# shaneson0/attacking_federate_learning

Measured on AMD Instinct MI355X. Metric: aggregation rounds/sec at N clients x D params (Bulyan), higher is better.
Workload: dtype f32 (Gram: fp16x2 split of every fp32 operand, 3 fp16 MFMAs per block, fp32/fp64 accumulate; <= 2e-7 of |gi||gj| vs f...

## Files before the change

### attacking_federate_learning_amd/_native.py

```python
import ctypes
import os

_HERE = os.path.dirname(os.path.abspath(__file__))
LIB_PATH = os.environ.get('BYZ_LIBRARY') or os.path.join(_HERE, 'libbyzagg.so')

OK, E_INVALID, E_PRECONDITION, E_HIP, E_UNSUPPORTED, E_NO_WINNER, E_COLLECTIVE = 0, -1, -2, -3, -4, -5, -6

KERNELS = ('column_stats', 'gram_tile', 'gram_reduce', 'distances', 'row_sort', 'krum_argmin',
           'bulyan_loop', 'trimmed_mean', 'misc', 'plane_split')

c_i64, c_i32, c_int, c_f32, c_vp = ctypes.c_int64, ctypes.c_int32, ctypes.c_int, ctypes.c_float, ctypes.c_void_p
_P = ctypes.POINTER



class GeomedParams(ctypes.Structure):
    _fields_ = [('nu', ctypes.c_double), ('max_iter', c_i64), ('ftol', ctypes.c_double)]


class CclipParams(ctypes.Structure):
    _fields_ = [('tau', ctypes.c_double), ('iters', c_i64)]


SIGNGUARD_MAX_SAMPLES = 1024
# ... 59 lines not shown
    'byz_upload': [c_vp, c_vp, c_vp, c_i64, c_vp],
    'byz_download': [c_vp, c_vp, c_vp, c_i64, c_vp],
    'byz_upload_2d': [c_vp, c_vp, c_i64, c_vp, c_i64, c_i64, c_i64, c_vp],
    'byz_stream_sync': [c_vp, c_vp],
    'byz_no_defense_dev': [c_vp, c_vp, c_i64, c_i64, c_i64, c_vp, c_vp],
    'byz_pairwise_distances_dev': [c_vp, c_vp, c_i64, c_i64, c_i64, c_vp, c_vp],
    'byz_gram_dev': [c_vp, c_vp, c_i64, c_i64, c_i64, c_vp, c_vp],
    'byz_gram_share_dev': [c_vp, c_vp, c_i64, c_i64, c_i64, c_vp, c_int, c_int, c_vp, c_vp],
    'byz_gram_share_add_dev': [c_vp, c_vp, c_i64, c_i64, c_i64, c_vp, c_int, c_int, c_vp, c_vp],
    'byz_distances_from_gram_dev': [c_vp, c_vp, c_i64, c_vp, c_vp],
    'byz_near_pairs_count': [c_vp, _P(c_i64), c_vp],
    'byz_near_pairs_sqdist_dev': [c_vp, c_vp, c_i64, c_i64, c_i64, c_vp, c_vp, c_vp],
    'byz_near_pairs_apply_dev': [c_vp, c_vp, c_i64, c_vp, c_vp],
    'byz_ctx_check': [c_vp, c_vp],
    'byz_bulyan_rescored': [c_vp, _P(c_i64)],
    'byz_krum_select_dev': [c_vp, c_vp, c_i64, c_i64, c_i64, _P(c_i32), c_vp, c_vp],
    'byz_krum_dev': [c_vp, c_vp, c_i64, c_i64, c_i64, c_i64, c_i64, c_int, c_vp, _P(c_i32), c_vp],
    'byz_trimmed_mean_dev': [c_vp, c_vp, c_i64, c_i64, c_i64, c_vp, c_i64, c_vp, c_vp],
    'byz_coordinate_median_dev': [c_vp, c_vp, c_i64, c_i64, c_i64, c_vp, c_vp, c_vp],
    'byz_rank_trimmed_mean_dev': [c_vp, c_vp, c_i64, c_i64, c_i64, c_vp, c_i64, c_vp, c_vp],
    'byz_window_mean_dev': [c_vp, c_vp, c_i64, c_i64, c_i64, c_vp, c_vp, c_i64, c_vp, c_vp, c_vp],
    'byz_phocas_dev': [c_vp, c_vp, c_i64, c_i64, c_i64, c_vp, c_i64, c_vp, c_vp, c_vp, c_vp],
    'byz_trimmed_mean_redone': [c_vp, _P(c_i64), c_vp],
    'byz_bulyan_select_dev': [c_vp, c_vp, c_i64, c_i64, c_i64, c_vp, c_vp],
    'byz_krum_bulyan_select_dev': [c_vp, c_vp, c_i64, c_i64, c_i64, _P(c_i32), c_vp, c_vp],
    'byz_bulyan_dev': [c_vp, c_vp, c_i64, c_i64, c_i64, c_i64, c_i64, c_vp, c_vp, c_vp],
    'byz_mean_rows_dev': [c_vp, c_vp, c_i64, c_i64, c_i64, c_vp, c_i64, c_vp, c_vp],
    'byz_multi_krum_select_dev': [c_vp, c_vp, c_i64, c_i64, c_i64, c_i64, c_vp, c_vp],
    'byz_multi_krum_dev': [c_vp, c_vp, c_i64, c_i64, c_i64, c_i64, c_i64, c_i64, c_int, c_vp, c_vp, c_vp],
    'byz_pairwise_distances_sharded_dev': [c_vp, c_vp, c_i64, c_i64, c_i64, c_vp, c_vp, c_vp, c_vp],
# ... 191 lines not shown
```

### attacking_federate_learning_amd/csrc/api.hip

```cpp
#include "common.hpp"

#include <cmath>
#include <cstring>

namespace byz {

static thread_local char g_error[1024] = "";

void set_error(const char* fmt, ...) {
    va_list ap;
    va_start(ap, fmt);
    vsnprintf(g_error, sizeof(g_error), fmt, ap);
    va_end(ap);
}

namespace {

int64_t python_prefix_len(int64_t length, int64_t stop) {
    if (stop >= 0) return stop < length ? stop : length;
    return length + stop > 0 ? length + stop : 0;
}

int enter(byz_ctx* ctx) {
    if (!ctx) {
// ... 190 lines not shown
    if (theta < 0 || theta > n) {
        set_error("bulyan: selection size %lld does not fit %lld rows", (long long)theta, (long long)n);
        return BYZ_E_INVALID;
    }
    int64_t drop = (n - 1) - users_count + corrupted;
    if (drop < 0) drop = 0;
    if (drop > n - 1) drop = n - 1;
    const int64_t krum_prefix = krum_winner_dev != nullptr ? python_prefix_len(n - 1, users_count - corrupted) : 0;
    BYZ_TRY(launch_row_sort(ctx, dist, n, krum_prefix, drop, true, stream));
    if (krum_winner_dev != nullptr) BYZ_TRY(launch_krum_argmin(ctx, n, krum_winner_dev, stream));
    BYZ_TRY(launch_bulyan_loop(ctx, dist, n, theta, drop, users_count, corrupted, selection_dev, &device_scalars(ctx)->core.bulyan, stream));
    CoreScalars core;
    BYZ_TRY(read_core(ctx, &core, stream));
    const int32_t status = core.bulyan.status;
    ctx->bulyan_rescored = core.bulyan.rescored;
    if (status == 2) {
        set_error("bulyan: the selection loop's workgroups lost contact with each other (exchange timed out)");
        return BYZ_E_HIP;
    }
    if (status != 0) {
        set_error("bulyan: no row scored below 1e20 (the reference raises KeyError(-1) here)");
        return BYZ_E_NO_WINNER;
    }
    return BYZ_OK;
}

int check_multi_krum_m(int64_t n, int64_t m) {
    if (m < 1 || m > n) {
        set_error("multi_krum: m = %lld outside 1..%lld (the row count)", (long long)m, (long long)n);
        return BYZ_E_INVALID;
// ... 280 lines not shown
    BYZ_REQUIRE(sq_dev && dist && n_rows > 0 && ctx->near_pair_capacity > 0, "near_pairs_apply: bad arguments");
    return launch_near_pair_apply(ctx, sq_dev, n_rows, dist, as_stream(stream));
}

int byz_ctx_check(byz_ctx* ctx, void* stream) {
    BYZ_TRY(enter(ctx));
    return check_core(ctx, as_stream(stream));
}

int byz_bulyan_rescored(const byz_ctx* ctx, int64_t* rows_host) {
    if (!ctx || !rows_host) {
        set_error("bulyan_rescored: null argument");
        return BYZ_E_INVALID;
    }
    *rows_host = ctx->bulyan_rescored;
    return BYZ_OK;
}

int byz_pairwise_distances_dev(byz_ctx* ctx, const float* G, int64_t n_rows, int64_t n_cols, int64_t ld,
                               float* dist, void* stream) {
    BYZ_TRY(enter(ctx));
    BYZ_TRY(check_matrix(G, n_rows, n_cols, ld, "pairwise_distances"));
    BYZ_REQUIRE(dist, "pairwise_distances: null output");
    return distances(ctx, G, n_rows, n_cols, ld, nullptr, nullptr, dist, stream);
}

int byz_krum_select_dev(byz_ctx* ctx, const float* dist, int64_t n_rows, int64_t users_count,
                        int64_t corrupted_count, int32_t* index_host, float* scores_dev, void* stream) {
    BYZ_TRY(enter(ctx));
    BYZ_REQUIRE(dist && n_rows > 0, "krum_select: bad arguments");
// ... 2532 lines not shown
```

### attacking_federate_learning_amd/csrc/common.hpp

```cpp
#pragma once

#include <hip/hip_runtime.h>

#include <cstdarg>
#include <cstdint>
#include <cstdio>
#include <cstdlib>
#include <string>
#include <unordered_map>
#include <vector>

#include "../../include/byzagg.h"
#include "carve.hpp"
#include "device_scalars.hpp"

namespace byz {

void set_error(const char* fmt, ...);

#define BYZ_HIP(expr)                                                                       \
    do {                                                                                    \
        hipError_t e_ = (expr);                                                             \
        if (e_ != hipSuccess) {                                                             \
            ::byz::set_error("%s failed: %s (%s:%d)", #expr, hipGetErrorString(e_), __FILE__, \
// ... 130 lines not shown
    int64_t fang_steps = 0, fang_chosen = -1;
    int32_t fang_succeeded = 0;
    byz::Buffer phocas;
    byz::Buffer large_keys;
    byz::Buffer large_idx;
    byz::Buffer large_rank;
    byz::Buffer large_rank_t;
    byz::Buffer large_dist_t;
    byz::Buffer large_state;
    byz::Buffer large_grid;
    bool redo_valid = false;
    byz::Buffer redo_tiles;
    byz::Buffer twin_class;
    byz::Buffer xchg;
    int64_t bulyan_rescored = 0;
    byz::Buffer selection;
    byz::Buffer scalars;
    byz::LastCall last[byz::kReportCount];
    bool small_configured = false;
    std::unordered_map<const void*, int> dynamic_lds;
    byz::Buffer assemble_table;
    std::vector<int64_t> assemble_host;
    hipEvent_t assemble_copied = nullptr;
    int64_t assemble_clients = 0, assemble_segments = 0, assemble_longest = 0, assemble_total = 0;
    byz::Buffer stage_in;
    byz::Buffer stage_out;
    byz::PinnedBuffer pinned;
    bool timing = false;
    byz::TimingSlot slots[BYZ_K_COUNT];
};
// ... 325 lines not shown
```

### attacking_federate_learning_amd/csrc/device_scalars.hpp

```cpp
#pragma once

#include <hip/hip_runtime.h>

#include <cstddef>
#include <cstdint>
#include <type_traits>

namespace byz {

constexpr int kStatusLostTicket = 1;
constexpr int kStatusPairOverflow = 2;
constexpr int kStatusFalseTwin = 4;
constexpr int kStatusSmallTimeout = 8;
constexpr int kStatusNoTurn = 16;

struct BulyanStatus { int32_t status, rescored, pad; };
struct CoreScalars {
    int32_t krum_winner, pad0[7];
    BulyanStatus bulyan;
    int32_t pad1[5];
    int32_t status;
    int32_t near_pairs;
    int32_t attack_redo, pad2;
};
struct GeomedReport {
    int32_t done, iterations, excluded, fallback;
    double objective;
};
struct DncReport { int32_t kept, inactive; };
struct CclipReport { int32_t clipped, excluded; };
struct FltrustReport {
// ... 108 lines not shown
```

### attacking_federate_learning_amd/csrc/select.hip

```cpp
#include "common.hpp"
#include "lane_exchange.hpp"
#include "order_keys.hpp"

#include <cstdlib>
#include <cstring>

namespace byz {
namespace {

using namespace lanes;

constexpr int kMaxSelectRows = 16384;
constexpr float kKrumInit = 1e20f;

__device__ __forceinline__ float integer_passes(uint32_t (&M)[8], const int (&ex)[8], float s, int lane);

__device__ __forceinline__ int sort_slot(int i) { return i + (i >> 4); }

__device__ __forceinline__ double key_to_double(uint32_t ordered, uint32_t column) {
    return static_cast<double>((static_cast<unsigned long long>(ordered) << 16) | column);
}
__device__ __forceinline__ unsigned long long double_to_key(double d) {
    const unsigned long long x = static_cast<unsigned long long>(d);
    return ((x >> 16) << 32) | (x & 0xffffull);
// ... 728 lines not shown
    int u, bad, ptr, alive;

    __device__ __forceinline__ void init(int row, int n, int drop, const double* __restrict__ row_total, const double* __restrict__ row_top,
                                         const uint16_t* __restrict__ rank_t, float* sorted_val) {
        u = row;
        alive = u < n;
        tot = alive ? row_total[u] : 0.0;
        top = (alive && drop > 0) ? row_top[u] : 0.0;
        bad = alive ? static_cast<int>(row_top[n + u]) : 0;
        ptr = n - 1 - drop;
        if (alive) sorted_val[static_cast<int64_t>(u) * n + rank_t[static_cast<int64_t>(u) * n + u]] = __uint_as_float(kGoneBits);
    }

    __device__ __forceinline__ void remove(int w, int n, int drop, const float* __restrict__ dist, const uint16_t* __restrict__ sorted_idx,
                                           const uint16_t* __restrict__ rank_t, const uint32_t* removed) {
        if (!alive) return;
        if (u == w) {
            alive = 0;
            return;
        }
        const float dwf = dist[static_cast<int64_t>(w) * n + u];
        const bool dw_finite = __builtin_fabsf(dwf) <= 3.4028234663852886e38f;
        const double dw = dw_finite ? static_cast<double>(dwf) : 0.0;
        if (!dw_finite) --bad;
        const int r = rank_t[static_cast<int64_t>(w) * n + u];
        tot -= dw;
        if (drop > 0 && r >= ptr) {
            top -= dw;
            int p = ptr - 1;
            const uint16_t* order = sorted_idx + static_cast<int64_t>(u) * n;
            while (p >= 0) {
                const int col = order[p];
                if (!((removed[col >> 5] >> (col & 31)) & 1u)) break;
                --p;
            }
            if (p >= 0) {
                const float joins = dist[static_cast<int64_t>(u) * n + order[p]];
                if (__builtin_fabsf(joins) <= 3.4028234663852886e38f) top += static_cast<double>(joins);
            }
            ptr = p;
        }
    }
};

__global__ __launch_bounds__(kGridThreads) void bulyan_grid_kernel(
    const float* __restrict__ dist, int n, int theta, int drop, int users_count, int corrupted,
    const uint16_t* __restrict__ sorted_idx, const uint16_t* __restrict__ rank_t, float* sorted_val,
    const double* __restrict__ row_total, const double* __restrict__ row_top, const int32_t* __restrict__ cls,
// ... 196 lines not shown
                    }
                    ptr = p;
                }
            }
        }
    }
    if (tid == 0) {
        if (result != 0) atomicMax(status, result);
        if (n_rescored) atomicAdd(rescored, n_rescored);
    }
}


constexpr int kSpecMax = 32;
constexpr int kSpecTable = 512;

__global__ __launch_bounds__(kGridThreads) void spec_owner_kernel(const double* __restrict__ row_total, const double* __restrict__ row_top,
                                                                  const int32_t* __restrict__ cls, int n, int drop, int n_wgs,
                                                                  int32_t* __restrict__ owner) {
    static_assert(kGridThreads == 256, "four waves per workgroup");
    __shared__ double tile[kGridThreads];
    __shared__ int copy[kGridThreads];
    __shared__ int sums[3][64];
    const int tid = threadIdx.x, lane = tid & 63, part = tid >> 6;
    const int u = blockIdx.x * 64 + lane;
    auto first_score = [&](int v) -> double {
        if (v >= n) return __builtin_inf();
        const double s = row_total[v] - (drop > 0 ? row_top[v] : 0.0);
        return s == s ? s : __builtin_inf();
    };
    const double su = first_score(u);
    const bool u_copy = u < n && cls[u] != u;
    int rank = 0, copies = 0, copies_before = 0;
    if (tid < 64) sums[0][tid] = sums[1][tid] = sums[2][tid] = 0;
    for (int v0 = 0; v0 < n; v0 += kGridThreads) {
        tile[tid] = first_score(v0 + tid);
        copy[tid] = (v0 + tid < n && cls[v0 + tid] != v0 + tid) ? 1 : 0;
        __syncthreads();
        const int m = n - v0 < kGridThreads ? n - v0 : kGridThreads;
        const int j_end = 64 * part + 64 < m ? 64 * part + 64 : m;
#pragma unroll 8
        for (int j = 64 * part; j < j_end; ++j) {
            const double sv = tile[j];
            const int cj = copy[j];
            copies += cj;
            copies_before += (cj != 0 && v0 + j < u) ? 1 : 0;
            rank += (cj == 0 && (sv < su || (sv == su && v0 + j < u))) ? 1 : 0;
        }
        __syncthreads();
    }
    atomicAdd(&sums[0][lane], rank);
    atomicAdd(&sums[1][lane], copies);
    atomicAdd(&sums[2][lane], copies_before);
    __syncthreads();
    if (part != 0 || u >= n) return;
    rank = sums[0][lane];
    copies = sums[1][lane];
    copies_before = sums[2][lane];
    if (u_copy) {
        owner[copies_before] = u;
        return;
    }
    const int q = copies / kGridThreads, rem = copies % kGridThreads;
    const int narrow = n_wgs - q - 1, wide = n_wgs - q;
    const int first_part = rem * narrow;
    int wg, local;
    if (rank < first_part) {
        local = rank / narrow;
        wg = q + 1 + rank % narrow;
    } else {
        const int r = rank - first_part;
        local = rem + r / wide;
        wg = q + r % wide;
    }
    owner[wg * kGridThreads + local] = u;
}

struct SpecVerdict {
    int k_bad;
    int winner;
    int timeout;
};

template <int kSpecThreads>
__global__ __launch_bounds__(kSpecThreads) void bulyan_spec_kernel(
    const float* __restrict__ dist, int n, int theta, int drop, int users_count, int corrupted,
    const uint16_t* __restrict__ sorted_idx, const uint16_t* __restrict__ rank_t, float* sorted_val,
    const double* __restrict__ row_total, const double* __restrict__ row_top, const int32_t* __restrict__ cls,
    unsigned long long* __restrict__ xchg, int32_t* __restrict__ selection, int32_t* __restrict__ status,
    int32_t* __restrict__ rescored, int batch_picks, const int32_t* __restrict__ owner) {
    __shared__ __attribute__((aligned(16))) float rescore_stage[kSpecThreads / 64][512];
    __shared__ Candidate slots[kSpecThreads / 64];
    __shared__ double second_slots[kSpecThreads / 64];
    __shared__ uint32_t removed[kMaxSelectRows / 32];
    __shared__ __attribute__((aligned(16))) uint32_t egone[kSpecThreads / 64][kMaxSelectRows / 32];
    __shared__ GridDecision decision;
    __shared__ int decision_contested;
    __shared__ unsigned long long leader_of[kSpecTable];
    __shared__ uint16_t items[kGridThreads * kSpecMax];
    __shared__ int n_items;
    __shared__ Candidate wave_bests[kSpecThreads / 64][kSpecMax];
    __shared__ int winners[kSpecMax];
    __shared__ SpecVerdict verdict;
    __shared__ int true_row[kSpecMax];
    __shared__ uint16_t front_batches[kGridThreads];
    const int tid = threadIdx.x, lane = tid & 63, wave = tid >> 6;
    const int n_wgs = gridDim.x, wg = blockIdx.x;
    const int u = tid < kGridThreads ? owner[wg * kGridThreads + tid] : n;
    for (int i = tid; i < kMaxSelectRows / 32; i += kSpecThreads) {
        removed[i] = 0u;
#pragma unroll
        for (int w = 0; w < kSpecThreads / 64; ++w) egone[w][i] = 0u;
    }
    if (tid < kGridThreads) front_batches[tid] = 0;

    BulyanRow row;
    row.init(u, n, drop, row_total, row_top, rank_t, sorted_val);
    const int my_class = row.alive ? cls[u] : 0;
    const int my_pos = visit_position(u);
    int n_rescored = 0;
    __syncthreads();

    auto slot = [&](int parity, int kind) { return xchg + (parity * 3 + kind) * kGridMaxWgs; };
    auto batch_slot = [&](int parity, int k) { return xchg + (6 + parity * kSpecMax + k) * kGridMaxWgs; };
    const unsigned long long none_a = (static_cast<unsigned long long>(kInfBits) << 32) | (static_cast<unsigned long long>(kNoRow) << 18);

    auto remove_winner = [&](int w) __attribute__((always_inline)) {
        if (tid == 0) removed[w >> 5] |= 1u << (w & 31);
        __syncthreads();
        row.remove(w, n, drop, dist, sorted_idx, rank_t, removed);
    };

    int result = (n < 2 && theta > 0) ? 1 : 0;
    int t = 0;
    uint32_t seq = 0;
    uint32_t batch_seq = 0;
    while (t < theta && result == 0) {
        const BulyanRow snapshot = row;
        const int t0 = t;
        const int kmax = theta - t0 < batch_picks ? theta - t0 : batch_picks;
        uint32_t cmask = 0;
        uint32_t contested = 0;
        int n_done = 0, pending = 0;
        for (int k = 0; k < kmax; ++k, ++seq) {
            const int tt = t0 + k;
            const uint32_t tag = ((seq >> 1) & 7u) + 1u;
            const uint32_t tag18 = (seq + 1u) & 0x3ffffu;
            const int parity = static_cast<int>(seq & 1u);
            const int take = take_at(tt, n, users_count, corrupted);
            const double score = row.tot - row.top;
            const bool candidate = row.alive && row.bad <= drop && score < static_cast<double>(kKrumInit);
            Candidate c{static_cast<double>(kKrumInit), 0x7fffffff, -1, -1};
            if (candidate) c = Candidate{score, my_pos, u, my_class};
            const Candidate best = block_best_dpp(c, slots);
            const int best_class = best.cls;
            double second = (candidate && my_class != best_class) ? score : __builtin_inf();
            second = wave_min_dpp(second);
            if (lane == 0) second_slots[wave] = second;
            __syncthreads();
// ... 10 lines not shown
                unsigned long long gb = static_cast<unsigned long long>(__float_as_uint(b_lb)) << 32;
                bool ok = true;
                if (n_wgs > 1) {
                    if (lane == 0) {
                        granule_store(slot(parity, 0) + wg, ga | tag);
                        granule_store(slot(parity, 1) + wg, gb | tag18);
                    }
                    unsigned long long va = none_a, vb = static_cast<unsigned long long>(kInfBits) << 32;
                    ok = gather_granule_pair(slot(parity, 0), slot(parity, 1), n_wgs, tag, tag18, lane, va, vb);
                    ga = va;
                    gb = vb;
                } else if (lane != 0) {
                    ga = none_a;
                    gb = static_cast<unsigned long long>(kInfBits) << 32;
                }
                const float a = __uint_as_float(static_cast<uint32_t>(ga >> 32));
                const float b = __uint_as_float(static_cast<uint32_t>(gb >> 32));
                const int a_row = static_cast<int>((ga >> 18) & 0x3fffu);
                const int a_cls = static_cast<int>((ga >> 4) & 0x3fffu);
                const float m1 = wave_min_dpp(a);
                GridDecision d{0, -1, 0.0};
                int is_contested = 0;
                if (!ok) {
                    d.mode = 3;
                } else if (!(m1 < __builtin_inff())) {
                    d.mode = 2;
                } else {
                    const double thr = band_threshold(m1, take);
                    d.threshold = thr;
                    const bool in_a = static_cast<double>(a) <= thr;
                    const bool in_b = static_cast<double>(b) <= thr;
                    const unsigned long long first = __ballot(a == m1);
                    const int lead_cls = __builtin_amdgcn_readlane(a_cls, __builtin_ctzll(first));
                    const bool one_class = __ballot(in_b) == 0ull && __ballot(in_a && a_cls != lead_cls) == 0ull;
                    const int pos = wave_min_dpp((one_class ? in_a : a == m1) ? visit_position(a_row) : 0x7fffffff);
                    d.winner = row_of_visit(pos);
                    is_contested = one_class ? 0 : 1;
                }
                if (lane == 0) {
                    decision = d;
                    decision_contested = is_contested;
                }
            }
            __syncthreads();
            const GridDecision d = decision;
            if (d.mode == 3) {
                result = 2;
                break;
            }
            if (d.mode == 2) {
                pending = 1;
                ++seq;
                break;
            }
            if (decision_contested != 0) {
                contested |= 1u << k;
                if (candidate && score <= d.threshold) cmask |= 1u << k;
            }
            if (tid == 0) winners[k] = d.winner;
            remove_winner(d.winner);
            ++n_done;
        }
        if (result != 0) break;
        contested &= n_done >= 32 ? ~0u : (1u << n_done) - 1u;
        cmask &= contested;

        int k_bad = -1, w_true = -1;
        if (contested != 0u) {
            for (int i = tid; i < kSpecTable; i += kSpecThreads) leader_of[i] = ~0ull;
            if (tid == 0) n_items = 0;
            if (tid < (kSpecThreads / 64) * kSpecMax)
                (&wave_bests[0][0])[tid] = Candidate{static_cast<double>(kKrumInit), 0x7fffffff, -1, -1};
            __syncthreads();
            for (uint32_t m = cmask; m != 0u; m &= m - 1u) {
                const int k = __builtin_ctz(m);
                const unsigned long long key = (static_cast<unsigned long long>(my_pos) << 32) | (static_cast<uint32_t>(k) << 16) | static_cast<uint32_t>(my_class);
// ... 104 lines not shown
                    }
                    verdict = v;
                }
                __syncthreads();
            }
            ++batch_seq;
            if (verdict.timeout != 0) {
                result = 2;
                break;
            }
            k_bad = verdict.k_bad;
            w_true = verdict.winner;
        }
        if (k_bad >= 0) {
            row = snapshot;
            __syncthreads();
            if (tid == 0) {
                for (int k = 0; k < n_done; ++k) removed[winners[k] >> 5] &= ~(1u << (winners[k] & 31));
                if (w_true >= 0) winners[k_bad] = w_true;
            }
            __syncthreads();
            n_done = w_true >= 0 ? k_bad + 1 : k_bad;
            pending = w_true >= 0 ? 0 : 1;
            for (int k = 0; k < n_done; ++k) remove_winner(winners[k]);
        }
        __syncthreads();
        for (int k = 0; k < n_done; ++k) {
            const int w = winners[k];
            if (wg == 0 && tid == 0) selection[t0 + k] = w;
            if (row.alive) sorted_val[static_cast<int64_t>(u) * n + rank_t[static_cast<int64_t>(w) * n + u]] = __uint_as_float(kGoneBits);
        }
        t = t0 + n_done;
        if (pending != 0) result = 1;
        __syncthreads();
    }
    if (tid == 0) {
        if (result != 0) atomicMax(status, result);
        if (n_rescored) atomicAdd(rescored, n_rescored);
    }
}

}

int64_t select_max_rows() { return kLargeMaxRows; }

bool select_large_applies(int64_t n) {
    if (n > kMaxSelectRows) return true;
    const char* e = std::getenv("BYZ_SELECT_LARGE");
    return e != nullptr && std::atoi(e) != 0;
}

int launch_row_sort(byz_ctx* ctx, const float* dist, int64_t n, int64_t prefix_len, int64_t drop_count,
                    bool want_tables, hipStream_t stream) {
// ... 47 lines not shown
    return check_launch("row_sort_kernel");
}

int launch_krum_argmin(byz_ctx* ctx, int64_t n, int32_t* winner_dev, hipStream_t stream) {
    KernelTimer t(ctx, BYZ_K_KRUM_ARGMIN, stream);
    krum_argmin_kernel<<<1, 1024, 0, stream>>>(ctx->scores.as<float>(), (int)n, winner_dev);
    return check_launch("krum_argmin_kernel");
}

int launch_bulyan_loop(byz_ctx* ctx, const float* dist, int64_t n, int64_t theta, int64_t drop_count,
                       int64_t users_count, int64_t corrupted, int32_t* selection_dev, BulyanStatus* status_dev,
                       hipStream_t stream) {
    BYZ_REQUIRE(dist && selection_dev && status_dev && n > 0 && theta >= 0 && theta <= n,
                "bulyan loop: bad arguments (n=%lld theta=%lld)", (long long)n, (long long)theta);
    BYZ_TRY(ctx->twin_class.ensure(static_cast<size_t>(2 * n) * sizeof(int32_t)));
    constexpr size_t kGranules = static_cast<size_t>(2 * 3 + 2 * kSpecMax) * kGridMaxWgs;
    BYZ_TRY(ctx->xchg.ensure(kGranules * sizeof(unsigned long long)));
    int32_t* cls_tmp = ctx->twin_class.as<int32_t>();
    int32_t* cls = cls_tmp + n;
    BYZ_HIP(hipMemsetAsync(ctx->xchg.ptr, 0, kGranules * sizeof(unsigned long long), stream));
    BYZ_HIP(hipMemsetAsync(status_dev, 0, sizeof *status_dev, stream));
    KernelTimer t(ctx, BYZ_K_BULYAN_LOOP, stream);
    twin_class_kernel<<<static_cast<unsigned>(ceil_div(n, 4)), 256, 0, stream>>>(dist, (int)n, cls_tmp);
    BYZ_TRY(check_launch("twin_class_kernel"));
    twin_class_fix_kernel<<<static_cast<unsigned>(ceil_div(n, 256)), 256, 0, stream>>>(cls_tmp, (int)n, cls);
    BYZ_TRY(check_launch("twin_class_fix_kernel"));
    if (select_large_applies(n))
        return launch_bulyan_loop_large(ctx, dist, n, theta, drop_count, users_count, corrupted, cls, selection_dev, status_dev, stream);
    const unsigned n_wgs = static_cast<unsigned>(ceil_div(n, kGridThreads));
    int batch = n >= 6000 ? 16 : (n >= 1000 ? 32 : 0);
    if (const char* e = std::getenv("BYZ_BULYAN_BATCH")) batch = std::atoi(e);
    if (batch > kSpecMax) batch = kSpecMax;
    if (batch >= 1) {
        BYZ_TRY(ctx->spec_owner.ensure(static_cast<size_t>(n_wgs) * kGridThreads * sizeof(int32_t)));
        int32_t* owner = ctx->spec_owner.as<int32_t>();
        BYZ_HIP(hipMemsetD32Async(reinterpret_cast<hipDeviceptr_t>(owner), static_cast<int>(n), static_cast<size_t>(n_wgs) * kGridThreads, stream));
        spec_owner_kernel<<<static_cast<unsigned>(ceil_div(n, 64)), kGridThreads, 0, stream>>>(
            ctx->row_total.as<double>(), ctx->row_top.as<double>(), cls, (int)n, (int)drop_count, (int)n_wgs, owner);
        BYZ_TRY(check_launch("spec_owner_kernel"));
        auto* spec = n >= 6000 ? &bulyan_spec_kernel<512> : &bulyan_spec_kernel<256>;
        spec<<<n_wgs, n >= 6000 ? 512 : 256, 0, stream>>>(
            dist, (int)n, (int)theta, (int)drop_count, (int)users_count, (int)corrupted, ctx->sorted_idx.as<uint16_t>(),
            ctx->rank_t.as<uint16_t>(), ctx->sorted_val.as<float>(), ctx->row_total.as<double>(), ctx->row_top.as<double>(), cls,
            ctx->xchg.as<unsigned long long>(), selection_dev, &status_dev->status, &status_dev->rescored, batch, owner);
        return check_launch("bulyan_spec_kernel");
    }
    bulyan_grid_kernel<<<n_wgs, kGridThreads, 0, stream>>>(
        dist, (int)n, (int)theta, (int)drop_count, (int)users_count, (int)corrupted, ctx->sorted_idx.as<uint16_t>(),
        ctx->rank_t.as<uint16_t>(), ctx->sorted_val.as<float>(), ctx->row_total.as<double>(), ctx->row_top.as<double>(), cls,
        ctx->xchg.as<unsigned long long>(), selection_dev, &status_dev->status, &status_dev->rescored);
    return check_launch("bulyan_grid_kernel");
}

}
```

### attacking_federate_learning_amd/engine.py

```python
import ctypes
import itertools
import os

import numpy as np

from . import _native

NAME_TO_ID = {'NoDefense': 0, 'Krum': 1, 'TrimmedMean': 2, 'Bulyan': 3}


def dnc_columns(n_cols, sub_dim, n_iters=1, seed=0):
    n_cols, sub_dim, n_iters = int(n_cols), int(sub_dim), int(n_iters)
    if n_iters < 1 or sub_dim < 1 or n_cols < 1:
        raise ValueError('dnc_columns: n_iters, sub_dim and n_cols must be >= 1')
    rng = np.random.default_rng(seed)
    rows = []
    for _ in range(n_iters):
        if sub_dim >= n_cols:
            rows.append(np.arange(n_cols, dtype=np.int64))
        else:
            rows.append(np.sort(rng.choice(n_cols, sub_dim, replace=False)).astype(np.int64))
    return np.stack(rows)


# ... 709 lines not shown

    def krum_bulyan_select(self, distances, users_count, corrupted_count, on_device=False):
        theta = int(users_count) - 2 * int(corrupted_count)
        with _Call(self) as c:
            d, keys = c.distances(distances)
            sel = DeviceBuffer(self, (max(theta, 1),), np.int32)
            idx = ctypes.c_int32(-2)
            c.run(self.lib.byz_krum_bulyan_select_dev(self.ctx, d.ptr, d.n, int(users_count), int(corrupted_count),
                                                      ctypes.byref(idx), sel.ptr, None), reads_back=True)
            index = int(idx.value)
            index = index if (keys is None or index < 0) else keys[index]
            return index, self._selection(sel, theta, keys, on_device)

    def bulyan_rescored(self):
        return self._read(self.lib.byz_bulyan_rescored, [ctypes.c_int64])[0]

    def bulyan(self, g, users_count, corrupted_count, return_selection=False):
        assert users_count >= 4 * corrupted_count + 3
        dm = self._device_matrix(g)
        if dm is None:
            if return_selection:
                out, aux = self.defend_host('Bulyan', g, users_count, corrupted_count, want_aux=True)
                return out, aux[:int(users_count) - 2 * int(corrupted_count)]
            return self.defend_host('Bulyan', g, users_count, corrupted_count)
        theta = int(users_count) - 2 * int(corrupted_count)
        with _Call(self) as c:
            m = c.matrix(dm)
            out, ptr = c.out(m.cols)
            sel, sel_ptr = c.out(max(theta, 1), np.int32, want=return_selection)
            c.run(self.lib.byz_bulyan_dev(self.ctx, m.ptr, m.rows, m.cols, m.ld, int(users_count), int(corrupted_count), ptr,
# ... 1587 lines not shown
```

### include/byzagg.h

```cpp
#ifndef BYZAGG_H
#define BYZAGG_H

#include <stdint.h>

#ifdef __cplusplus
extern "C" {
#endif

#define BYZ_ABI_VERSION 1

enum {
    BYZ_OK = 0,
    BYZ_E_INVALID = -1,
    BYZ_E_PRECONDITION = -2,
    BYZ_E_HIP = -3,
    BYZ_E_UNSUPPORTED = -4,
    BYZ_E_NO_WINNER = -5,
    BYZ_E_COLLECTIVE = -6
};

typedef struct byz_ctx byz_ctx;

int byz_abi_version(void);
const char* byz_last_error(void);
// ... 53 lines not shown
                              float* out_dev, void* stream);

int byz_window_mean_dev(byz_ctx* ctx, const float* G_dev, int64_t n_rows, int64_t n_cols, int64_t ld,
                        const int32_t* row_index_dev, const float* centre_dev, int64_t keep,
                        float* out_dev, float* radius_dev, void* stream);
int byz_phocas_dev(byz_ctx* ctx, const float* G_dev, int64_t n_rows, int64_t n_cols, int64_t ld,
                   const int32_t* row_index_dev, int64_t trim_count, float* out_dev,
                   float* centre_out_dev, float* radius_dev, void* stream);

int byz_bulyan_select_dev(byz_ctx* ctx, const float* dist_dev, int64_t n_rows, int64_t users_count,
                          int64_t corrupted_count, int32_t* selection_dev, void* stream);
int byz_krum_bulyan_select_dev(byz_ctx* ctx, const float* dist_dev, int64_t n_rows, int64_t users_count,
                               int64_t corrupted_count, int32_t* krum_index_host, int32_t* selection_dev,
                               void* stream);
int byz_bulyan_rescored(const byz_ctx* ctx, int64_t* rows_host);
int byz_bulyan_dev(byz_ctx* ctx, const float* G_dev, int64_t n_rows, int64_t n_cols, int64_t ld,
                   int64_t users_count, int64_t corrupted_count, float* out_dev,
                   int32_t* selection_dev, void* stream);

int byz_mean_rows_dev(byz_ctx* ctx, const float* G_dev, int64_t n_rows, int64_t n_cols, int64_t ld,
                      const int32_t* row_index_dev, int64_t count, float* out_dev, void* stream);
int byz_multi_krum_select_dev(byz_ctx* ctx, const float* dist_dev, int64_t n_rows, int64_t users_count,
                              int64_t corrupted_count, int64_t m, int32_t* selection_dev, void* stream);
int byz_multi_krum_dev(byz_ctx* ctx, const float* G_dev, int64_t n_rows, int64_t n_cols, int64_t ld,
                       int64_t users_count, int64_t corrupted_count, int64_t m, int check_assert,
                       float* out_dev, int32_t* selection_dev, void* stream);

#define BYZ_GEOMED_MAX_ITER 65536
typedef struct byz_geomed_params {
    double nu;
// ... 418 lines not shown
```

Measured before the change: 2.126.

## Predict Bulyan selection runs from first-round score order and verify them speculatively

Precomputes a predicted pick order by ranking rows on their initial Krum scores, then in the Bulyan selection loop takes runs of predicted winners and checks them all in one grid exchange instead of one exchange per pick. Mispredictions cut the run short, and an adaptive stretch falls back to one-by-one picking after poor runs. The aim is fewer cross-workgroup synchronisations per selected row, paid for with extra replay work, more LDS and exchange slots, and a more complex rollback path.

```diff
diff --git a/attacking_federate_learning_amd/_native.py b/attacking_federate_learning_amd/_native.py
--- a/attacking_federate_learning_amd/_native.py
+++ b/attacking_federate_learning_amd/_native.py
@@ -97,6 +97,7 @@
     'byz_near_pairs_apply_dev': [c_vp, c_vp, c_i64, c_vp, c_vp],
     'byz_ctx_check': [c_vp, c_vp],
     'byz_bulyan_rescored': [c_vp, _P(c_i64)],
+    'byz_bulyan_predicted': [c_vp, _P(c_i64), _P(c_i64)],
     'byz_krum_select_dev': [c_vp, c_vp, c_i64, c_i64, c_i64, _P(c_i32), c_vp, c_vp],
     'byz_krum_dev': [c_vp, c_vp, c_i64, c_i64, c_i64, c_i64, c_i64, c_int, c_vp, _P(c_i32), c_vp],
     'byz_trimmed_mean_dev': [c_vp, c_vp, c_i64, c_i64, c_i64, c_vp, c_i64, c_vp, c_vp],
diff --git a/attacking_federate_learning_amd/csrc/api.hip b/attacking_federate_learning_amd/csrc/api.hip
--- a/attacking_federate_learning_amd/csrc/api.hip
+++ b/attacking_federate_learning_amd/csrc/api.hip
@@ -228,6 +228,7 @@
     BYZ_TRY(read_core(ctx, &core, stream));
     const int32_t status = core.bulyan.status;
     ctx->bulyan_rescored = core.bulyan.rescored;
+    ctx->bulyan_predicted = core.bulyan.predicted;
     if (status == 2) {
         set_error("bulyan: the selection loop's workgroups lost contact with each other (exchange timed out)");
         return BYZ_E_HIP;
@@ -538,6 +539,16 @@
         return BYZ_E_INVALID;
     }
     *rows_host = ctx->bulyan_rescored;
+    return BYZ_OK;
+}
+
+int byz_bulyan_predicted(const byz_ctx* ctx, int64_t* runs_host, int64_t* picks_host) {
+    if (!ctx || !runs_host || !picks_host) {
+        set_error("bulyan_predicted: null argument");
+        return BYZ_E_INVALID;
+    }
+    *runs_host = static_cast<uint32_t>(ctx->bulyan_predicted) >> 16;
+    *picks_host = ctx->bulyan_predicted & 0xffff;
     return BYZ_OK;
 }
 
diff --git a/attacking_federate_learning_amd/csrc/common.hpp b/attacking_federate_learning_amd/csrc/common.hpp
--- a/attacking_federate_learning_amd/csrc/common.hpp
+++ b/attacking_federate_learning_amd/csrc/common.hpp
@@ -168,6 +168,7 @@
     byz::Buffer twin_class;
     byz::Buffer xchg;
     int64_t bulyan_rescored = 0;
+    int32_t bulyan_predicted = 0;
     byz::Buffer selection;
     byz::Buffer scalars;
     byz::LastCall last[byz::kReportCount];
diff --git a/attacking_federate_learning_amd/csrc/device_scalars.hpp b/attacking_federate_learning_amd/csrc/device_scalars.hpp
--- a/attacking_federate_learning_amd/csrc/device_scalars.hpp
+++ b/attacking_federate_learning_amd/csrc/device_scalars.hpp
@@ -14,7 +14,7 @@
 constexpr int kStatusSmallTimeout = 8;
 constexpr int kStatusNoTurn = 16;
 
-struct BulyanStatus { int32_t status, rescored, pad; };
+struct BulyanStatus { int32_t status, rescored, predicted; };
 struct CoreScalars {
     int32_t krum_winner, pad0[7];
     BulyanStatus bulyan;
diff --git a/attacking_federate_learning_amd/csrc/select.hip b/attacking_federate_learning_amd/csrc/select.hip
--- a/attacking_federate_learning_amd/csrc/select.hip
+++ b/attacking_federate_learning_amd/csrc/select.hip
@@ -766,24 +766,30 @@
 
     __device__ __forceinline__ void remove(int w, int n, int drop, const float* __restrict__ dist, const uint16_t* __restrict__ sorted_idx,
                                            const uint16_t* __restrict__ rank_t, const uint32_t* removed) {
+        if (!alive || u == w) return remove_loaded(w, 0.0f, 0, n, drop, dist, sorted_idx, [](int) { return false; });
+        const float dwf = dist[static_cast<int64_t>(w) * n + u];
+        const int r = rank_t[static_cast<int64_t>(w) * n + u];
+        remove_loaded(w, dwf, r, n, drop, dist, sorted_idx, [removed](int col) { return ((removed[col >> 5] >> (col & 31)) & 1u) != 0u; });
+    }
+
+    template <typename Gone>
+    __device__ __forceinline__ void remove_loaded(int w, float dwf, int r, int n, int drop, const float* __restrict__ dist,
+                                                  const uint16_t* __restrict__ sorted_idx, Gone gone) {
         if (!alive) return;
         if (u == w) {
             alive = 0;
             return;
         }
-        const float dwf = dist[static_cast<int64_t>(w) * n + u];
         const bool dw_finite = __builtin_fabsf(dwf) <= 3.4028234663852886e38f;
         const double dw = dw_finite ? static_cast<double>(dwf) : 0.0;
         if (!dw_finite) --bad;
-        const int r = rank_t[static_cast<int64_t>(w) * n + u];
         tot -= dw;
         if (drop > 0 && r >= ptr) {
             top -= dw;
             int p = ptr - 1;
             const uint16_t* order = sorted_idx + static_cast<int64_t>(u) * n;
             while (p >= 0) {
-                const int col = order[p];
-                if (!((removed[col >> 5] >> (col & 31)) & 1u)) break;
+                if (!gone(static_cast<int>(order[p]))) break;
                 --p;
             }
             if (p >= 0) {
@@ -1010,14 +1016,25 @@
 
 constexpr int kSpecMax = 32;
 constexpr int kSpecTable = 512;
+constexpr int kPredStretch = 8, kPredStretchMax = 256;
+constexpr int kPredFirst = 8;
+constexpr int kPredChunk = 8;
+
+template <int I, int N, typename F>
+__device__ __forceinline__ void static_for(F&& f) {
+    if constexpr (I < N) {
+        f(std::integral_constant<int, I>{});
+        static_for<I + 1, N>(f);
+    }
+}
 
 __global__ __launch_bounds__(kGridThreads) void spec_owner_kernel(const double* __restrict__ row_total, const double* __restrict__ row_top,
                                                                   const int32_t* __restrict__ cls, int n, int drop, int n_wgs,
-                                                                  int32_t* __restrict__ owner) {
+                                                                  int32_t* __restrict__ owner, int32_t* __restrict__ pred_order) {
     static_assert(kGridThreads == 256, "four waves per workgroup");
     __shared__ double tile[kGridThreads];
     __shared__ int copy[kGridThreads];
-    __shared__ int sums[3][64];
+    __shared__ int sums[4][64];
     const int tid = threadIdx.x, lane = tid & 63, part = tid >> 6;
     const int u = blockIdx.x * 64 + lane;
     auto first_score = [&](int v) -> double {
@@ -1027,8 +1044,9 @@
     };
     const double su = first_score(u);
     const bool u_copy = u < n && cls[u] != u;
-    int rank = 0, copies = 0, copies_before = 0;
-    if (tid < 64) sums[0][tid] = sums[1][tid] = sums[2][tid] = 0;
+    const int u_pos = visit_position(u);
+    int rank = 0, copies = 0, copies_before = 0, rank_all = 0;
+    if (tid < 64) sums[0][tid] = sums[1][tid] = sums[2][tid] = sums[3][tid] = 0;
     for (int v0 = 0; v0 < n; v0 += kGridThreads) {
         tile[tid] = first_score(v0 + tid);
         copy[tid] = (v0 + tid < n && cls[v0 + tid] != v0 + tid) ? 1 : 0;
@@ -1042,14 +1060,17 @@
             copies += cj;
             copies_before += (cj != 0 && v0 + j < u) ? 1 : 0;
             rank += (cj == 0 && (sv < su || (sv == su && v0 + j < u))) ? 1 : 0;
+            rank_all += (sv < su || (sv == su && visit_position(v0 + j) < u_pos)) ? 1 : 0;
         }
         __syncthreads();
     }
     atomicAdd(&sums[0][lane], rank);
     atomicAdd(&sums[1][lane], copies);
     atomicAdd(&sums[2][lane], copies_before);
+    atomicAdd(&sums[3][lane], rank_all);
     __syncthreads();
     if (part != 0 || u >= n) return;
+    pred_order[sums[3][lane]] = u;
     rank = sums[0][lane];
     copies = sums[1][lane];
     copies_before = sums[2][lane];
@@ -1078,13 +1099,49 @@
     int timeout;
 };
 
-template <int kSpecThreads>
+__device__ __forceinline__ GridDecision decide_optimistic(unsigned long long ga, unsigned long long gb, bool ok, int take, int& is_contested) {
+    const float a = __uint_as_float(static_cast<uint32_t>(ga >> 32));
+    const float b = __uint_as_float(static_cast<uint32_t>(gb >> 32));
+    const int a_row = static_cast<int>((ga >> 18) & 0x3fffu);
+    const int a_cls = static_cast<int>((ga >> 4) & 0x3fffu);
+    const float m1 = wave_min_dpp(a);
+    GridDecision d{0, -1, 0.0};
+    is_contested = 0;
+    if (!ok) {
+        d.mode = 3;
+    } else if (!(m1 < __builtin_inff())) {
+        d.mode = 2;
+    } else {
+        const double thr = band_threshold(m1, take);
+        d.threshold = thr;
+        const bool in_a = static_cast<double>(a) <= thr;
+        const bool in_b = static_cast<double>(b) <= thr;
+        const unsigned long long first = __ballot(a == m1);
+        const int lead_cls = __builtin_amdgcn_readlane(a_cls, __builtin_ctzll(first));
+        const bool one_class = __ballot(in_b) == 0ull && __ballot(in_a && a_cls != lead_cls) == 0ull;
+        const int pos = wave_min_dpp((one_class ? in_a : a == m1) ? visit_position(a_row) : 0x7fffffff);
+        d.winner = row_of_visit(pos);
+        is_contested = one_class ? 0 : 1;
+    }
+    return d;
+}
+
+template <int kWaves>
+struct PredictedShared {
+    double second[kSpecMax][kWaves];
+    unsigned long long pub_a[kSpecMax], pub_b[kSpecMax];
+    double threshold[kSpecMax];
+    int mode[kSpecMax], winner[kSpecMax], contested[kSpecMax];
+};
+
+template <int kSpecThreads, bool kPredict>
 __global__ __launch_bounds__(kSpecThreads) void bulyan_spec_kernel(
     const float* __restrict__ dist, int n, int theta, int drop, int users_count, int corrupted,
     const uint16_t* __restrict__ sorted_idx, const uint16_t* __restrict__ rank_t, float* sorted_val,
     const double* __restrict__ row_total, const double* __restrict__ row_top, const int32_t* __restrict__ cls,
     unsigned long long* __restrict__ xchg, int32_t* __restrict__ selection, int32_t* __restrict__ status,
-    int32_t* __restrict__ rescored, int batch_picks, const int32_t* __restrict__ owner) {
+    int32_t* __restrict__ rescored, int batch_picks, const int32_t* __restrict__ owner, const int32_t* __restrict__ pred_order,
+    int32_t* __restrict__ predicted) {
     __shared__ __attribute__((aligned(16))) float rescore_stage[kSpecThreads / 64][512];
     __shared__ Candidate slots[kSpecThreads / 64];
     __shared__ double second_slots[kSpecThreads / 64];
@@ -1092,7 +1149,15 @@
     __shared__ __attribute__((aligned(16))) uint32_t egone[kSpecThreads / 64][kMaxSelectRows / 32];
     __shared__ GridDecision decision;
     __shared__ int decision_contested;
-    __shared__ unsigned long long leader_of[kSpecTable];
+    __shared__ union {
+        unsigned long long leader_of[kSpecTable];
+        PredictedShared<kGridThreads / 64> predicted;
+    } phase;
+    static_assert(sizeof(PredictedShared<kGridThreads / 64>) <= sizeof(unsigned long long) * kSpecTable, "the predicted picks' LDS fits the leaders' table");
+    unsigned long long* const leader_of = phase.leader_of;
+    auto& ps = phase.predicted;
+    __shared__ int pred[kSpecMax];
+    __shared__ int pred_len, pred_skip;
     __shared__ uint16_t items[kGridThreads * kSpecMax];
     __shared__ int n_items;
     __shared__ Candidate wave_bests[kSpecThreads / 64][kSpecMax];
@@ -1119,6 +1184,7 @@
 
     auto slot = [&](int parity, int kind) { return xchg + (parity * 3 + kind) * kGridMaxWgs; };
     auto batch_slot = [&](int parity, int k) { return xchg + (6 + parity * kSpecMax + k) * kGridMaxWgs; };
+    auto pred_slot = [&](int parity, int kind, int k) { return xchg + (6 + 2 * kSpecMax + (parity * 2 + kind) * kSpecMax + k) * kGridMaxWgs; };
     const unsigned long long none_a = (static_cast<unsigned long long>(kInfBits) << 32) | (static_cast<unsigned long long>(kNoRow) << 18);
 
     auto remove_winner = [&](int w) __attribute__((always_inline)) {
@@ -1131,14 +1197,208 @@
     int t = 0;
     uint32_t seq = 0;
     uint32_t batch_seq = 0;
+    uint32_t pred_seq = 0;
+    int pred_cursor = 0;
+    int pred_picks = kPredFirst, one_by_one = 0, stretch = kPredStretch;
+    int n_runs = 0, run_picks = 0;
     while (t < theta && result == 0) {
         const BulyanRow snapshot = row;
+        const int cursor_snapshot = pred_cursor;
         const int t0 = t;
         const int kmax = theta - t0 < batch_picks ? theta - t0 : batch_picks;
         uint32_t cmask = 0;
         uint32_t contested = 0;
         int n_done = 0, pending = 0;
-        for (int k = 0; k < kmax; ++k, ++seq) {
+        int k = 0;
+        while (k < kmax) {
+            if (kPredict && __builtin_expect(one_by_one == 0, 0)) {
+                if (wave == 0) {
+                    const int want = kmax - k < pred_picks ? kmax - k : pred_picks;
+                    const int at = pred_cursor + lane;
+                    const int cand = at < n ? pred_order[at] : -1;
+                    const bool live = cand >= 0 && cand < n && ((removed[cand >> 5] >> (cand & 31)) & 1u) == 0u;
+                    const unsigned long long live_mask = __ballot(live);
+                    const int before = __popcll(live_mask & ((1ull << lane) - 1ull));
+                    if (live && before < want) pred[before] = cand;
+                    if (lane == 0) {
+                        const int found = __popcll(live_mask);
+                        pred_len = found < want ? found : want;
+                        pred_skip = live_mask != 0ull ? __builtin_ctzll(live_mask) : (n - pred_cursor < 64 ? (n - pred_cursor > 0 ? n - pred_cursor : 0) : 64);
+                    }
+                }
+                __syncthreads();
+                const int len = pred_len;
+                pred_cursor += pred_skip;
+                if (len == 0) {
+                    one_by_one = 1;
+                    __syncthreads();
+                    continue;
+                }
+                const uint32_t ptag = ((pred_seq >> 1) & 7u) + 1u;
+                const uint32_t ptag18 = (pred_seq + 1u) & 0x3ffffu;
+                const int ppar = static_cast<int>(pred_seq & 1u);
+                auto gone_behind = [&](int j) {
+                    return [&, j](int col) {
+                        if (((removed[col >> 5] >> (col & 31)) & 1u) != 0u) return true;
+                        for (int i = 0; i <= j; ++i)
+                            if (pred[i] == col) return true;
+                        return false;
+                    };
+                };
+                struct Loaded {
+                    float dist[kPredChunk];
+                    uint32_t rank[kPredChunk / 2];
+                    __device__ __forceinline__ int rank_of(int i) const { return static_cast<int>((rank[i / 2] >> (16 * (i % 2))) & 0xffffu); }
+                };
+                auto load_chunk = [&](int j0, int count) {
+                    Loaded c;
+                    static_for<0, kPredChunk>([&](auto ic) {
+                        constexpr int i = decltype(ic)::value;
+                        c.dist[i] = 0.0f;
+                        if (i % 2 == 0) c.rank[i / 2] = 0u;
+                        if (j0 + i < count && row.alive) {
+                            const int64_t at = static_cast<int64_t>(pred[j0 + i]) * n + u;
+                            c.dist[i] = dist[at];
+                            c.rank[i / 2] |= static_cast<uint32_t>(rank_t[at]) << (16 * (i % 2));
+                        }
+                    });
+                    return c;
+                };
+                if (tid < kGridThreads) {
+                    BulyanRow replay = row;
+                    Loaded next = load_chunk(0, len);
+                    for (int j0 = 0; j0 < len; j0 += kPredChunk) {
+                        const Loaded now = next;
+                        next = load_chunk(j0 + kPredChunk, len);
+                        static_for<0, kPredChunk>([&](auto ic) {
+                            constexpr int i = decltype(ic)::value;
+                            const int j = j0 + i;
+                            if (j < len) {
+                                const double score = replay.tot - replay.top;
+                                const bool candidate = replay.alive && replay.bad <= drop && score < static_cast<double>(kKrumInit);
+                                const double low = wave_min_dpp(candidate ? score : __builtin_inf());
+                                unsigned long long holds = __ballot(candidate && score == low);
+                                if (__popcll(holds) > 1) {
+                                    const int first_pos = wave_min_dpp((candidate && score == low) ? my_pos : 0x7fffffff);
+                                    holds = __ballot(candidate && score == low && my_pos == first_pos);
+                                }
+                                Candidate wave_best{static_cast<double>(kKrumInit), 0x7fffffff, -1, -1};
+                                if (holds != 0ull) {
+                                    const int from = __builtin_ctzll(holds);
+                                    wave_best = Candidate{low, readlane(my_pos, from), readlane(u, from), readlane(my_class, from)};
+                                }
+                                const double second = wave_min_dpp((candidate && my_class != wave_best.cls) ? score : __builtin_inf());
+                                if (lane == 0) {
+                                    wave_bests[wave][j] = wave_best;
+                                    ps.second[j][wave] = second;
+                                }
+                                replay.remove_loaded(pred[j], now.dist[i], now.rank_of(i), n, drop, dist, sorted_idx, gone_behind(j));
+                            }
+                        });
+                    }
+                }
+                __syncthreads();
+                if (wave == 0) {
+                    const int j = lane & (kSpecMax - 1);
+                    unsigned long long ga = none_a, gb = static_cast<unsigned long long>(kInfBits) << 32;
+                    if (j < len) {
+                        Candidate best = wave_bests[0][j];
+#pragma unroll
+                        for (int w = 1; w < kGridThreads / 64; ++w)
+                            if (better(wave_bests[w][j], best)) best = wave_bests[w][j];
+                        double sec = __builtin_inf();
+#pragma unroll
+                        for (int w = 0; w < kGridThreads / 64; ++w) {
+                            const Candidate o = wave_bests[w][j];
+                            sec = fmin(sec, o.cls == best.cls ? ps.second[j][w] : (o.row >= 0 ? o.score : __builtin_inf()));
+                        }
+                        if (best.row >= 0)
+                            ga = (static_cast<unsigned long long>(__float_as_uint(float_below(best.score))) << 32) |
+                                 (static_cast<unsigned long long>(best.row) << 18) | (static_cast<unsigned long long>(best.cls) << 4);
+                        gb = static_cast<unsigned long long>(__float_as_uint(float_below(sec))) << 32;
+                    }
+                    if (lane < kSpecMax) {
+                        ps.pub_a[j] = ga;
+                        if (n_wgs > 1) granule_store(pred_slot(ppar, 0, j) + wg, ga | ptag);
+                    } else {
+                        ps.pub_b[j] = gb;
+                        if (n_wgs > 1) granule_store(pred_slot(ppar, 1, j) + wg, gb | ptag18);
+                    }
+                }
+                __syncthreads();
+                for (int j = wave; j < len; j += kSpecThreads / 64) {
+                    unsigned long long ga = none_a, gb = static_cast<unsigned long long>(kInfBits) << 32;
+                    bool ok = true;
+                    if (n_wgs > 1) {
+                        ok = gather_granule_pair(pred_slot(ppar, 0, j), pred_slot(ppar, 1, j), n_wgs, ptag, ptag18, lane, ga, gb);
+                    } else if (lane == 0) {
+                        ga = ps.pub_a[j];
+                        gb = ps.pub_b[j];
+                    }
+                    int is_contested = 0;
+                    const GridDecision d = decide_optimistic(ga, gb, ok, take_at(t0 + k + j, n, users_count, corrupted), is_contested);
+                    if (lane == 0) {
+                        ps.mode[j] = d.mode;
+                        ps.winner[j] = d.winner;
+                        ps.threshold[j] = d.threshold;
+                        ps.contested[j] = is_contested;
+                    }
+                }
+                __syncthreads();
+                ++pred_seq;
+                const bool mine = lane < len;
+                if (__ballot(mine && ps.mode[mine ? lane : 0] == 3) != 0ull) {
+                    result = 2;
+                    break;
+                }
+                const unsigned long long missed = __ballot(mine && (ps.mode[mine ? lane : 0] != 0 || ps.winner[mine ? lane : 0] != pred[mine ? lane : 0]));
+                const int cut = missed != 0ull ? __builtin_ctzll(missed) : len;
+                const bool nobody = cut < len && ps.mode[cut < len ? cut : 0] == 2;
+                const int cut_winner = (cut < len && !nobody) ? ps.winner[cut] : -1;
+                const int committed = cut + (cut_winner >= 0 ? 1 : 0);
+                for (int j0 = 0; j0 < committed; j0 += kPredChunk) {
+                    const Loaded now = load_chunk(j0, cut);
+                    static_for<0, kPredChunk>([&](auto ic) {
+                        constexpr int i = decltype(ic)::value;
+                        const int j = j0 + i;
+                        if (j < committed) {
+                            if (ps.contested[j] != 0) {
+                                const double score = row.tot - row.top;
+                                const bool candidate = row.alive && row.bad <= drop && score < static_cast<double>(kKrumInit);
+                                contested |= 1u << (k + j);
+                                if (candidate && score <= ps.threshold[j]) cmask |= 1u << (k + j);
+                            }
+                            if (j < cut) row.remove_loaded(pred[j], now.dist[i], now.rank_of(i), n, drop, dist, sorted_idx, gone_behind(j));
+                        }
+                    });
+                }
+                __syncthreads();
+                if (tid == 0) {
+                    for (int j = 0; j < cut; ++j) {
+                        winners[k + j] = pred[j];
+                        removed[pred[j] >> 5] |= 1u << (pred[j] & 31);
+                    }
+                    if (cut_winner >= 0) winners[k + cut] = cut_winner;
+                }
+                if (cut_winner >= 0) remove_winner(cut_winner);
+                __syncthreads();
+                k += committed;
+                n_done += committed;
+                ++n_runs;
+                run_picks += committed;
+                if (nobody) {
+                    pending = 1;
+                    break;
+                }
+                if (11 * committed >= 31 + len) {
+                    stretch = kPredStretch;
+                } else {
+                    one_by_one = stretch;
+                    stretch = 2 * stretch < kPredStretchMax ? 2 * stretch : kPredStretchMax;
+                }
+                pred_picks = 2 * committed < kSpecMax ? (committed < 2 ? 4 : 2 * committed) : kSpecMax;
+                continue;
+            }
             const int tt = t0 + k;
             const uint32_t tag = ((seq >> 1) & 7u) + 1u;
             const uint32_t tag18 = (seq + 1u) & 0x3ffffu;
@@ -1179,29 +1439,8 @@
                     ga = none_a;
                     gb = static_cast<unsigned long long>(kInfBits) << 32;
                 }
-                const float a = __uint_as_float(static_cast<uint32_t>(ga >> 32));
-                const float b = __uint_as_float(static_cast<uint32_t>(gb >> 32));
-                const int a_row = static_cast<int>((ga >> 18) & 0x3fffu);
-                const int a_cls = static_cast<int>((ga >> 4) & 0x3fffu);
-                const float m1 = wave_min_dpp(a);
-                GridDecision d{0, -1, 0.0};
                 int is_contested = 0;
-                if (!ok) {
-                    d.mode = 3;
-                } else if (!(m1 < __builtin_inff())) {
-                    d.mode = 2;
-                } else {
-                    const double thr = band_threshold(m1, take);
-                    d.threshold = thr;
-                    const bool in_a = static_cast<double>(a) <= thr;
-                    const bool in_b = static_cast<double>(b) <= thr;
-                    const unsigned long long first = __ballot(a == m1);
-                    const int lead_cls = __builtin_amdgcn_readlane(a_cls, __builtin_ctzll(first));
-                    const bool one_class = __ballot(in_b) == 0ull && __ballot(in_a && a_cls != lead_cls) == 0ull;
-                    const int pos = wave_min_dpp((one_class ? in_a : a == m1) ? visit_position(a_row) : 0x7fffffff);
-                    d.winner = row_of_visit(pos);
-                    is_contested = one_class ? 0 : 1;
-                }
+                const GridDecision d = decide_optimistic(ga, gb, ok, take, is_contested);
                 if (lane == 0) {
                     decision = d;
                     decision_contested = is_contested;
@@ -1225,6 +1464,9 @@
             if (tid == 0) winners[k] = d.winner;
             remove_winner(d.winner);
             ++n_done;
+            ++k;
+            ++seq;
+            if (one_by_one > 0) --one_by_one;
         }
         if (result != 0) break;
         contested &= n_done >= 32 ? ~0u : (1u << n_done) - 1u;
@@ -1359,6 +1601,7 @@
         }
         if (k_bad >= 0) {
             row = snapshot;
+            pred_cursor = cursor_snapshot;
             __syncthreads();
             if (tid == 0) {
                 for (int k = 0; k < n_done; ++k) removed[winners[k] >> 5] &= ~(1u << (winners[k] & 31));
@@ -1382,6 +1625,7 @@
     if (tid == 0) {
         if (result != 0) atomicMax(status, result);
         if (n_rescored) atomicAdd(rescored, n_rescored);
+        if (wg == 0) *predicted = ((n_runs & 0x7fff) << 16) | (run_picks & 0xffff);
     }
 }
 
@@ -1459,7 +1703,7 @@
     BYZ_REQUIRE(dist && selection_dev && status_dev && n > 0 && theta >= 0 && theta <= n,
                 "bulyan loop: bad arguments (n=%lld theta=%lld)", (long long)n, (long long)theta);
     BYZ_TRY(ctx->twin_class.ensure(static_cast<size_t>(2 * n) * sizeof(int32_t)));
-    constexpr size_t kGranules = static_cast<size_t>(2 * 3 + 2 * kSpecMax) * kGridMaxWgs;
+    constexpr size_t kGranules = static_cast<size_t>(2 * 3 + 2 * kSpecMax + 4 * kSpecMax) * kGridMaxWgs;
     BYZ_TRY(ctx->xchg.ensure(kGranules * sizeof(unsigned long long)));
     int32_t* cls_tmp = ctx->twin_class.as<int32_t>();
     int32_t* cls = cls_tmp + n;
@@ -1476,18 +1720,23 @@
     int batch = n >= 6000 ? 16 : (n >= 1000 ? 32 : 0);
     if (const char* e = std::getenv("BYZ_BULYAN_BATCH")) batch = std::atoi(e);
     if (batch > kSpecMax) batch = kSpecMax;
+    int predict = 1;
+    if (const char* e = std::getenv("BYZ_BULYAN_PREDICT")) predict = std::atoi(e) != 0 ? 1 : 0;
     if (batch >= 1) {
-        BYZ_TRY(ctx->spec_owner.ensure(static_cast<size_t>(n_wgs) * kGridThreads * sizeof(int32_t)));
+        const size_t n_slots = static_cast<size_t>(n_wgs) * kGridThreads;
+        BYZ_TRY(ctx->spec_owner.ensure((n_slots + static_cast<size_t>(n)) * sizeof(int32_t)));
         int32_t* owner = ctx->spec_owner.as<int32_t>();
+        int32_t* pred_order = owner + n_slots;
         BYZ_HIP(hipMemsetD32Async(reinterpret_cast<hipDeviceptr_t>(owner), static_cast<int>(n), static_cast<size_t>(n_wgs) * kGridThreads, stream));
         spec_owner_kernel<<<static_cast<unsigned>(ceil_div(n, 64)), kGridThreads, 0, stream>>>(
-            ctx->row_total.as<double>(), ctx->row_top.as<double>(), cls, (int)n, (int)drop_count, (int)n_wgs, owner);
+            ctx->row_total.as<double>(), ctx->row_top.as<double>(), cls, (int)n, (int)drop_count, (int)n_wgs, owner, pred_order);
         BYZ_TRY(check_launch("spec_owner_kernel"));
-        auto* spec = n >= 6000 ? &bulyan_spec_kernel<512> : &bulyan_spec_kernel<256>;
+        auto* spec = n >= 6000 ? (predict ? &bulyan_spec_kernel<512, true> : &bulyan_spec_kernel<512, false>)
+                               : (predict ? &bulyan_spec_kernel<256, true> : &bulyan_spec_kernel<256, false>);
         spec<<<n_wgs, n >= 6000 ? 512 : 256, 0, stream>>>(
             dist, (int)n, (int)theta, (int)drop_count, (int)users_count, (int)corrupted, ctx->sorted_idx.as<uint16_t>(),
             ctx->rank_t.as<uint16_t>(), ctx->sorted_val.as<float>(), ctx->row_total.as<double>(), ctx->row_top.as<double>(), cls,
-            ctx->xchg.as<unsigned long long>(), selection_dev, &status_dev->status, &status_dev->rescored, batch, owner);
+            ctx->xchg.as<unsigned long long>(), selection_dev, &status_dev->status, &status_dev->rescored, batch, owner, pred_order, &status_dev->predicted);
         return check_launch("bulyan_spec_kernel");
     }
     bulyan_grid_kernel<<<n_wgs, kGridThreads, 0, stream>>>(
diff --git a/attacking_federate_learning_amd/engine.py b/attacking_federate_learning_amd/engine.py
--- a/attacking_federate_learning_amd/engine.py
+++ b/attacking_federate_learning_amd/engine.py
@@ -747,6 +747,9 @@
 
     def bulyan_rescored(self):
         return self._read(self.lib.byz_bulyan_rescored, [ctypes.c_int64])[0]
+
+    def bulyan_predicted(self):
+        return tuple(self._read(self.lib.byz_bulyan_predicted, [ctypes.c_int64, ctypes.c_int64]))
 
     def bulyan(self, g, users_count, corrupted_count, return_selection=False):
         assert users_count >= 4 * corrupted_count + 3
diff --git a/include/byzagg.h b/include/byzagg.h
--- a/include/byzagg.h
+++ b/include/byzagg.h
@@ -91,6 +91,7 @@
                                int64_t corrupted_count, int32_t* krum_index_host, int32_t* selection_dev,
                                void* stream);
 int byz_bulyan_rescored(const byz_ctx* ctx, int64_t* rows_host);
+int byz_bulyan_predicted(const byz_ctx* ctx, int64_t* runs_host, int64_t* picks_host);
 int byz_bulyan_dev(byz_ctx* ctx, const float* G_dev, int64_t n_rows, int64_t n_cols, int64_t ld,
                    int64_t users_count, int64_t corrupted_count, float* out_dev,
                    int32_t* selection_dev, void* stream);
```

New measurement: 2.138 (median of 6 runs). No clear change (+0.5%).
